# junipertcy/bipartiteSBM-MCMC

Measured on NVIDIA B200. Metric: vertex-moves/sec, higher is better.
Workload: dtype f64+int32

## Files before the change

### bipartitesbm-mcmc_b200/csrc/capi.cu

```cuda
#include "../../include/bisbm.h"

#include <cuda_runtime.h>
#include <dlfcn.h>
#include <nccl.h>

#include <algorithm>
#include <chrono>
#include <cmath>
#include <cstdarg>
#include <cstdio>
#include <cstdlib>
#include <cstring>
#include <map>
#include <set>
#include <memory>
#include <mutex>
#include <numeric>
#include <string>
#include <vector>

#include "ingest.cuh"
#include "replay.cuh"
#include "merge.cuh"
#include "gltable.h"
// ... 48 lines not shown

struct bisbm_handle {
    int device = 0;
    std::shared_ptr<GraphDev> gdev;
    cudaStream_t stream = nullptr;
    cudaEvent_t ev0 = nullptr, ev1 = nullptr;
    int sm_count = 148;
    uint32_t n = 0, na = 0, nb = 0, W = 0, max_degree = 0;
    uint64_t n_edges = 0;
    std::vector<uint32_t> h_row_ptr, h_degvals;
    uint32_t *d_row_ptr = nullptr, *d_col = nullptr, *d_degidx = nullptr;
    double ent_base = 0.0;
    double* d_qtab = nullptr;
    GlNode* d_gl = nullptr;
    uint32_t gl_n = 0;
    uint32_t qn = 0, qk = 0;
    double* d_lg = nullptr;
    uint64_t lg_n = 0;
    uint32_t n_chains = 0, C = 0, KA = 0, KB = 0;
    std::vector<uint32_t> h_ka, h_kb;
    uint32_t *d_ka = nullptr, *d_kb = nullptr;
    int32_t *d_labels = nullptr, *d_labels_tmp = nullptr, *d_m = nullptr, *d_e = nullptr, *d_nr = nullptr,
            *d_eta = nullptr;
    int32_t *d_m2 = nullptr, *d_e2 = nullptr, *d_nr2 = nullptr;
    int32_t* d_nr_live = nullptr;
    int32_t* d_eta_snap = nullptr;
    double* d_kat_out = nullptr;
    ncclComm_t comm = nullptr;
    uint8_t* d_lab8 = nullptr;
    double eps = 1.0;
    LogqExp* d_lq = nullptr;
    uint64_t* d_seeds = nullptr;
    uint8_t* d_active = nullptr;
    unsigned long long *d_accepted = nullptr, *d_u = nullptr, *d_sweeps = nullptr;
    double *d_dS = nullptr, *d_entmin = nullptr, *d_ent_out = nullptr;
    uint32_t* d_nactive = nullptr;
    uint64_t sweep_epoch = 0;
    std::map<uint32_t, ReplaySlot> replay;
    uint32_t* d_hist = nullptr;
    uint32_t hist_width = 0;
    uint32_t al_ka = 0, al_kb = 0, al_segments = 0;
    uint32_t *d_al_order = nullptr, *d_al_seg = nullptr, *d_al_overlap = nullptr, *d_al_map = nullptr;
    bool al_sampled = false;
    double last_ms = 0.0;
    uint64_t last_launches = 0, last_moves = 0;
    int precision = BISBM_PRECISION_FP64;
    int opt_kernel = -1;
    uint32_t opt_inflight_div = 64;
    int opt_generic = 0;
// ... 24 lines not shown
template <typename T>
void dfree(T*& p) {
    if (p) cudaFree(p);
    p = nullptr;
}

void free_ladder(bisbm_handle* h) {
    dfree(h->d_tp_rung_beta); dfree(h->d_tp_beta); dfree(h->d_tp_rung_of); dfree(h->d_tp_chain_at); dfree(h->d_tp_trip);
    dfree(h->d_tp_acc_prev); dfree(h->d_tp_stats);
    h->tp_rungs = 0;
    h->tp_round = 0;
}

void free_align(bisbm_handle* h) {
    dfree(h->d_al_order); dfree(h->d_al_seg); dfree(h->d_al_overlap); dfree(h->d_al_map);
    h->al_ka = h->al_kb = h->al_segments = 0;
    h->al_sampled = false;
}

void free_chains(bisbm_handle* h) {
    free_ladder(h);
    free_align(h);
    dfree(h->d_ka); dfree(h->d_kb); dfree(h->d_labels); dfree(h->d_labels_tmp);
    dfree(h->d_m); dfree(h->d_e); dfree(h->d_nr); dfree(h->d_eta); dfree(h->d_lq); dfree(h->d_m2); dfree(h->d_e2); dfree(h->d_nr2); dfree(h->d_nr_live); dfree(h->d_eta_snap); dfree(h->d_kat_out); dfree(h->d_lab8);
    dfree(h->d_seeds); dfree(h->d_active); dfree(h->d_accepted); dfree(h->d_u); dfree(h->d_sweeps);
    dfree(h->d_dS); dfree(h->d_entmin); dfree(h->d_ent_out); dfree(h->d_nactive); dfree(h->d_hist);
    for (auto& kv : h->replay) { dfree(kv.second.d_rs); dfree(kv.second.d_vlist); dfree(kv.second.d_kh); }
    h->replay.clear();
    h->n_chains = 0;
}

GraphView gview(const bisbm_handle* h) {
    GraphView g;
    g.n = h->n; g.na = h->na; g.nb = h->nb; g.n_edges = h->n_edges;
    g.row_ptr = h->d_row_ptr; g.col = h->d_col; g.degidx = h->d_degidx;
    g.W = h->W; g.max_degree = h->max_degree;
    return g;
}

StateView sview(const bisbm_handle* h) {
    StateView s;
    s.C = h->C; s.KA = h->KA; s.KB = h->KB; s.W = h->W;
    s.labels = h->d_labels; s.m = h->d_m; s.e = h->d_e; s.nr = h->d_nr; s.eta = h->d_eta;
    s.ka = h->d_ka; s.kb = h->d_kb; s.eps = h->eps;
    return s;
}

// ... 436 lines not shown
        if (e != cudaSuccess)
            return fail(BISBM_ERR_CUDA, "sweep_kernel launch failed: %s (kernel %d, grid %u, %d threads, %zu bytes of shared memory)",
                        cudaGetErrorString(e), lp.kernel, grid, NT, lp.smem_bytes);
    }
    return BISBM_OK;
}

template <typename HistT>
int launch_sweep_nt(bisbm_handle* h, const SweepParams& P, const LaunchPlan& lp) {
    if (lp.wpc == 32) return launch_sweep_t<HistT, 1024>(h, P, lp);
    return launch_sweep_t<HistT, 512>(h, P, lp);
}

int launch_sweep_h(bisbm_handle* h, const SweepParams& P, const LaunchPlan& lp) {
    if (lp.hist_bytes == 1) return launch_sweep_nt<uint8_t>(h, P, lp);
    if (lp.hist_bytes == 2) return launch_sweep_nt<uint16_t>(h, P, lp);
    return launch_sweep_nt<uint32_t>(h, P, lp);
}

template <typename R, int KF, int TYPE, bool STAGED = true, int NT = 512>
int launch_sweep2_t(bisbm_handle* h, const SweepParams& P, const LaunchPlan& lp, unsigned grid) {
    int rc = ensure_smem_attr(h, (const void*)sweep2_kernel<R, KF, TYPE, STAGED, NT>, (int)kSmemMax);
    if (rc) return rc;
    sweep2_kernel<R, KF, TYPE, STAGED, NT><<<grid, lp.wpc * 32, lp.smem_bytes, h->stream>>>(P);
    {
        const cudaError_t e = cudaGetLastError();
        if (e != cudaSuccess)
            return fail(BISBM_ERR_CUDA, "sweep2_kernel launch failed: %s (kernel %d, grid %u, %u warps, %zu bytes of shared memory)",
                        cudaGetErrorString(e), lp.kernel, grid, lp.wpc, lp.smem_bytes);
    }
    wrote_labels8(h);
    return BISBM_OK;
}

template <typename R>
int launch_sweep2(bisbm_handle* h, const SweepParams& P, const LaunchPlan& lp, unsigned grid) {
    if (!kern_is_s2(lp.kernel) || lp.wpc > 24) return fail(BISBM_ERR_STATE, "internal: sweep2 launcher with the plan of kernel %d (%u warps)", lp.kernel, lp.wpc);
    if (!lp.smem) return launch_sweep2_t<R, 0, 0, false>(h, P, lp, grid);
    if (h->KA == 32 && h->KB == 32 && !h->opt_generic) {
#ifdef BISBM_WARP_VARIANTS
        if (lp.wpc == 24) return P.type ? launch_sweep2_t<R, 32, 1, true, 768>(h, P, lp, grid) : launch_sweep2_t<R, 32, 0, true, 768>(h, P, lp, grid);
        if (lp.wpc == 20) return P.type ? launch_sweep2_t<R, 32, 1, true, 640>(h, P, lp, grid) : launch_sweep2_t<R, 32, 0, true, 640>(h, P, lp, grid);
#endif
        return P.type ? launch_sweep2_t<R, 32, 1>(h, P, lp, grid) : launch_sweep2_t<R, 32, 0>(h, P, lp, grid);
    }
    return launch_sweep2_t<R, 0, 0>(h, P, lp, grid);
}

__attribute__((noinline)) int dispatch_sweep(bisbm_handle* h, const SweepParams& P, const LaunchPlan& lp, unsigned grid) {
    switch (lp.kernel) {
        case KERN_S2_F64: case KERN_S2L_F64: return launch_sweep2<double>(h, P, lp, grid);
        case KERN_S2_F32: case KERN_S2L_F32: return launch_sweep2<float>(h, P, lp, grid);
        case KERN_L2: {
            const int rc = launch_sweep_h(h, P, lp);
            wrote_labels32(h);
            return rc;
        }
        default: return fail(BISBM_ERR_STATE, "internal: no launcher for kernel %d", lp.kernel);
    }
}

SweepParams base_params(bisbm_handle* h, uint32_t type) {
    SweepParams P;
    memset(&P, 0, sizeof P);
    P.g = gview(h); P.s = sview(h); P.tb = tview(h, false);
    P.lab8 = h->d_lab8; P.m_next = h->d_m2; P.e_next = h->d_e2; P.nr_next = h->d_nr2; P.nr_live = h->d_nr_live;
    P.eta_read = h->d_eta;
    P.seeds = h->d_seeds; P.active = h->d_active; P.accepted = h->d_accepted; P.dS_accum = h->d_dS;
    P.lq = h->d_lq;
    P.n_chains = h->n_chains; P.type = type; P.n_groups = h->C / 32;
    P.kopp_max = type ? h->KA : h->KB;
    P.half_bits = feistel_half_bits(type ? h->nb : h->na);
    P.kat_out = h->d_kat_out;
    P.vary_k = (uint32_t)h->opt_vary_k;
    return P;
}

int launch_full_sweep(bisbm_handle* h, int schedule, float p0, float p1, uint64_t sweep_in_call, uint32_t max_inflight,
                      const double* beta_chain = nullptr) {
    uint32_t wpc = 32;
    const int kernel = plan_kernel(h, &wpc);
    if (!kern_is_s2(kernel)) {
        int rc = sync_labels32(h);
        if (rc) return rc;
    }
    {
        int rc = sync_labels8(h);
        if (rc) return rc;
    }
    for (uint32_t type = 0; type < 2; ++type) {
        const uint32_t nv = type ? h->nb : h->na;
        if (nv == 0) continue;
        LaunchPlan lp;
        int rc = plan_sweep(h, type, max_inflight, kernel, wpc, &lp);
        if (rc) return rc;
        const uint32_t kmax = type ? h->KB : h->KA;
        const uint32_t tot = h->n_chains * kmax;
        logq_refresh_kernel<<<(tot * 16 + 127) / 128, 128, 0, h->stream>>>(sview(h), tview(h, false), h->d_lq, h->n_chains, type);
        h->last_launches += 1;
        const uint32_t n_m = h->C * h->KA * h->KB, n_e = h->C * (h->KA + h->KB);
        const bool sliced = lp.smem && lp.ctas_per_group > 1;
        h->last_wpc = lp.wpc; h->last_cpg = lp.ctas_per_group; h->last_slice = lp.slice;
        h->last_kernel = kernel;
        uint32_t extras = 0;
        const uint32_t G = h->C / 32;
        if (sliced && h->opt_spare_sms && max_inflight == 0 && (uint32_t)h->sm_count > G * lp.ctas_per_group)
            extras = std::min<uint32_t>((uint32_t)h->sm_count - G * lp.ctas_per_group, G - 1);
        const uint32_t per_cta = lp.slice / std::max<uint32_t>(1, lp.ctas_per_group);
        for (uint32_t l = 0;; ++l) {
            const uint64_t pos = extras ? ((uint64_t)l * lp.ctas_per_group + ((uint64_t)l * extras) / G) * per_cta : (uint64_t)l * lp.slice;
            if (pos >= nv) break;
            if (sliced && l != 0 && l % h->opt_logq_every == 0) {
                logq_refresh_kernel<<<(tot * 16 + 127) / 128, 128, 0, h->stream>>>(sview(h), tview(h, false), h->d_lq, h->n_chains, type, 1u);
                h->last_launches += 1;
            }
            if (sliced) {
                const uint32_t nmax = std::max(std::max(n_m, n_e), G * kmax * h->W * 32u);
                sweep2_preinit_kernel<<<(nmax + 255) / 256, 256, 0, h->stream>>>(h->d_m, h->d_e, h->d_nr, h->d_m2, h->d_e2, h->d_nr2,
                                                                                 h->d_nr_live, n_m, n_e, h->KA, h->KB, type, lp.ctas_per_group - 1,
                                                                                 G, extras, l, h->d_eta, h->d_eta_snap, h->W);
                h->last_launches += 1;
            }
            SweepParams P = base_params(h, type);
            if (sliced) P.eta_read = h->d_eta_snap;
            P.ctas_per_group = lp.ctas_per_group; P.warps_used = lp.warps_used;
            P.pos_begin = (uint32_t)pos; P.pos_end = (uint32_t)std::min<uint64_t>(nv, pos + lp.slice);
            P.exclusive = sliced ? 0 : 1;
            P.sweep = h->sweep_epoch;
            P.step_base = sweep_in_call * (uint64_t)h->n + (type ? h->na : 0);
            P.schedule = schedule; P.p0 = p0; P.p1 = p1; P.beta0 = (p0 == 0.0f) ? -1.0 : 1.0 / (double)p0;
            if (schedule == BISBM_ABRUPT_COOL) {
                const uint64_t lo = P.step_base, hi = P.step_base + nv;
                if ((float)(hi - 1) < p0) { P.schedule = BISBM_CONSTANT; P.p0 = 1.0f; P.beta0 = 1.0; }
                else if (!((float)lo < p0)) { P.schedule = BISBM_CONSTANT; P.p0 = 0.0f; P.beta0 = -1.0; }
            }
            P.beta_chain = beta_chain;
            P.extras = extras; P.launch_idx = l; P.per_cta = per_cta;
            const unsigned grid = P.n_groups * lp.ctas_per_group + extras;
            rc = dispatch_sweep(h, P, lp, grid);
            if (rc) return rc;
            h->last_launches += 1;
            h->last_sweep_launches += 1;
            if (sliced) {
                std::swap(h->d_m, h->d_m2); std::swap(h->d_e, h->d_e2); std::swap(h->d_nr, h->d_nr2);
            }
        }
    }
    h->sweep_epoch++;
    h->last_moves += (uint64_t)h->n * h->n_chains;
    return BISBM_OK;
}

int sync_labels8(bisbm_handle* h) {
    if (!h->lab8_stale) return BISBM_OK;
    const uint64_t total = (uint64_t)h->n * h->C;
    const uint64_t threads = (total + 3) / 4;
    labels8_kernel<<<(unsigned)((threads + 255) / 256), 256, 0, h->stream>>>(h->d_labels, h->d_lab8, total);
    CU(cudaGetLastError());
    h->lab8_stale = false;
    return BISBM_OK;
}

int sync_labels32(bisbm_handle* h) {
    if (!h->lab32_stale) return BISBM_OK;
    const uint64_t total = (uint64_t)h->n * h->C;
    const uint64_t threads = (total + 3) / 4;
    labels32_kernel<<<(unsigned)((threads + 255) / 256), 256, 0, h->stream>>>(h->d_lab8, h->d_labels, total);
    CU(cudaGetLastError());
// ... 221 lines not shown
    free_ladder(h);
    free_align(h);
    uint32_t KA = 0, KB = 0;
    for (uint32_t c = 0; c < n_chains; ++c) {
        if (ka[c] == 0 || kb[c] == 0) return fail(BISBM_ERR_ARG, "chain %u: ka and kb must be >= 1", c);
        KA = std::max(KA, ka[c]); KB = std::max(KB, kb[c]);
    }
    KA = std::max(KA, h->opt_reserve_ka); KB = std::max(KB, h->opt_reserve_kb);
    const uint32_t C = (n_chains + 31) / 32 * 32;
    const uint32_t n = h->n;
    const size_t KK = (size_t)KA + KB;
    bool reuse = h->n_chains == n_chains && h->C == C && h->KA == KA && h->KB == KB && h->d_labels;
    bool same_model = reuse && h->eps == eps;
    for (uint32_t c = 0; same_model && c < n_chains; ++c) same_model = h->h_ka[c] == ka[c] && h->h_kb[c] == kb[c];
    if (!reuse) {
        free_chains(h);
        h->n_chains = n_chains; h->C = C; h->KA = KA; h->KB = KB;
        CU(cudaMalloc(&h->d_ka, C * sizeof(uint32_t)));
        CU(cudaMalloc(&h->d_kb, C * sizeof(uint32_t)));
        CU(cudaMalloc(&h->d_labels, (size_t)n * C * sizeof(int32_t)));
        CU(cudaMalloc(&h->d_labels_tmp, (size_t)n * C * sizeof(int32_t)));
        CU(cudaMalloc(&h->d_m, (size_t)C * KA * KB * sizeof(int32_t)));
        CU(cudaMalloc(&h->d_e, (size_t)C * KK * sizeof(int32_t)));
        CU(cudaMalloc(&h->d_m2, (size_t)C * KA * KB * sizeof(int32_t)));
        CU(cudaMalloc(&h->d_e2, (size_t)C * KK * sizeof(int32_t)));
        CU(cudaMalloc(&h->d_lab8, (size_t)n * C));
        CU(cudaMalloc(&h->d_nr, (size_t)C * KK * sizeof(int32_t)));
        CU(cudaMalloc(&h->d_nr2, (size_t)C * KK * sizeof(int32_t)));
        CU(cudaMalloc(&h->d_nr_live, (size_t)C * KK * sizeof(int32_t)));
        CU(cudaMalloc(&h->d_kat_out, 2 * sizeof(double)));
        CU(cudaMalloc(&h->d_eta, (size_t)C * KK * h->W * sizeof(int32_t)));
        CU(cudaMalloc(&h->d_eta_snap, (size_t)C * KK * h->W * sizeof(int32_t)));
        CU(cudaMalloc(&h->d_lq, (size_t)C * KK * sizeof(LogqExp)));
        CU(cudaMalloc(&h->d_seeds, C * sizeof(uint64_t)));
        CU(cudaMalloc(&h->d_active, C));
        CU(cudaMalloc(&h->d_accepted, C * sizeof(unsigned long long)));
        CU(cudaMalloc(&h->d_u, C * sizeof(unsigned long long)));
        CU(cudaMalloc(&h->d_sweeps, C * sizeof(unsigned long long)));
        CU(cudaMalloc(&h->d_dS, C * sizeof(double)));
        CU(cudaMalloc(&h->d_entmin, C * sizeof(double)));
        CU(cudaMalloc(&h->d_ent_out, C * sizeof(double)));
        CU(cudaMalloc(&h->d_nactive, sizeof(uint32_t)));
    } else {
        for (auto& kv : h->replay) { dfree(kv.second.d_rs); dfree(kv.second.d_vlist); dfree(kv.second.d_kh); }
        h->replay.clear();
    }
    h->eps = eps;
    h->h_ka.assign(C, 1); h->h_kb.assign(C, 1);
    std::copy(ka, ka + n_chains, h->h_ka.begin());
    std::copy(kb, kb + n_chains, h->h_kb.begin());
    CU(cudaMemsetAsync(h->d_lq, 0, (size_t)C * KK * sizeof(LogqExp), h->stream));
    CU(cudaMemsetAsync(h->d_dS, 0, C * sizeof(double), h->stream));
    CU(cudaMemsetAsync(h->d_active, 0, C, h->stream));
    CU(cudaMemsetAsync(h->d_active, 1, n_chains, h->stream));
    CU(cudaMemcpyAsync(h->d_ka, h->h_ka.data(), C * sizeof(uint32_t), cudaMemcpyHostToDevice, h->stream));
// ... 1084 lines not shown
    } else if (k == "warps") {
        if (value != 16 && value != 20 && value != 24) return fail(BISBM_ERR_ARG, "warps: 16, 20 or 24");
        h->opt_warps = (uint32_t)value;
    } else if (k == "generic") {
        h->opt_generic = value != 0;
    } else if (k == "logq_every") {
        if (value < 1 || value > 0x7fffffff) return fail(BISBM_ERR_ARG, "logq_every must be >= 1");
        h->opt_logq_every = (uint32_t)value;
    } else if (k == "spare_sms") {
        h->opt_spare_sms = value != 0;
    } else if (k == "reserve_ka" || k == "reserve_kb") {
        if (value < 0 || value > (1 << 20)) return fail(BISBM_ERR_ARG, "%s out of range", name);
        (k == "reserve_ka" ? h->opt_reserve_ka : h->opt_reserve_kb) = (uint32_t)value;
    } else {
        return fail(BISBM_ERR_ARG, "unknown option '%s'", name);
    }
    return BISBM_OK;
}

#ifdef BISBM_ROUND_CLOCKS
int bisbm_round_clocks(unsigned long long* out) {
    if (!out) return fail(BISBM_ERR_ARG, "null argument");
    CU(cudaDeviceSynchronize());
    CU(cudaMemcpyFromSymbol(out, g_round_clocks, sizeof(unsigned long long) * 8));
    const unsigned long long zero[8] = {0, 0, 0, 0, 0, 0, 0, 0};
    CU(cudaMemcpyToSymbol(g_round_clocks, zero, sizeof zero));
    return BISBM_OK;
}
#endif

int bisbm_parallel_transition(bisbm_handle* h, uint32_t chain, uint32_t v, uint32_t s, double* dS, double* log_accu) {
    int rc = need_chains(h);
    if (rc) return rc;
    if (chain >= h->n_chains) return fail(BISBM_ERR_ARG, "chain %u out of range", chain);
    const uint32_t ka = h->h_ka[chain], kb = h->h_kb[chain];
    if (v >= h->n || s >= ka + kb) return fail(BISBM_ERR_ARG, "vertex or block out of range");
    const bool va = v < h->na;
    if ((s < ka) != va) {
        if (dS) *dS = INFINITY;
        if (log_accu) *log_accu = NAN;
        return BISBM_OK;
    }
    uint32_t wpc = 32;
    const int kernel = plan_kernel(h, &wpc);
    if (!kern_is_s2(kernel))
        return fail(BISBM_ERR_STATE, "bisbm_parallel_transition needs the sweep2 kernel (degrees > 255 or K > 256 per type take the round-1 kernel)");
    const uint32_t type = va ? 0 : 1;
    rc = sync_labels8(h);
// ... 320 lines not shown
```

### bipartitesbm-mcmc_b200/csrc/sweep.cuh

```cuda
#pragma once
#include "state.cuh"

namespace bisbm {

struct LogqExp {
    int32_t e0, n0;
    double fe, fn;
    float fee, fen, fnn, feee;
    uint32_t valid, pad;
};

struct SweepParams {
    GraphView g;
    StateView s;
    Tables tb;
    uint8_t* lab8;
    int32_t* m_next;
    int32_t* e_next;
    const uint64_t* seeds;
    const uint8_t* active;
    unsigned long long* accepted;
    double* dS_accum;
    const LogqExp* lq;
    uint32_t n_chains;
    uint32_t type;
    uint32_t n_groups;
    uint32_t ctas_per_group;
    uint32_t warps_used;
    uint32_t pos_begin, pos_end;
    uint32_t half_bits;
    uint32_t kopp_max;
    uint32_t exclusive;
    uint64_t sweep;
    uint64_t step_base;
    int schedule;
    float p0, p1;
    int32_t* nr_next;
    int32_t* nr_live;
    const int32_t* eta_read;
    uint32_t group_offset;
    uint32_t kat_mode;
    uint32_t kat_chain, kat_v, kat_s;
    double* kat_out;
    double beta0;
    uint32_t extras, launch_idx, per_cta;
    uint32_t vary_k;
    const double* beta_chain;
};

BISBM_NOINLINE_HD static double par_temperature(int schedule, float p0, float p1, uint64_t t) {
    switch (schedule) {
        case 0: return (double)p0 * pow((double)p1, (double)t);
        case 1: return (double)(p0 - p1 * (float)t);
        case 2: {
            uint64_t i = (uint64_t)((float)t + p1);
            double l = (i == 0) ? 0.0 : log((double)i);
            return (double)p0 / l;
        }
        case 3: return (double)p0;
        default: return ((float)t < p0) ? 1.0 : 0.0;
    }
}
// ... 440 lines not shown
```

### bipartitesbm-mcmc_b200/csrc/sweep2.cuh

```cuda
#pragma once
#include <string.h>
#include "sweep.cuh"

namespace bisbm {

#if !defined(BISBM_NO_CVT_MAGIC) && !defined(BISBM_CVT_MAGIC)
#define BISBM_CVT_MAGIC 1
#endif

#define BISBM_LN2F 0.69314718055994530942f
#define BISBM_LOG2EF 1.44269504088896340736f

#if defined(__CUDA_ARCH__)
__device__ __forceinline__ float f_lg2(float x) { float y; asm("lg2.approx.ftz.f32 %0, %1;" : "=f"(y) : "f"(x)); return y; }
__device__ __forceinline__ float f_ex2(float x) { float y; asm("ex2.approx.ftz.f32 %0, %1;" : "=f"(y) : "f"(x)); return y; }
__device__ __forceinline__ float f_rcp(float x) { float y; asm("rcp.approx.ftz.f32 %0, %1;" : "=f"(y) : "f"(x)); return y; }
#else
inline float f_lg2(float x) { return log2f(x); }
inline float f_ex2(float x) { return exp2f(x); }
inline float f_rcp(float x) { return 1.0f / x; }
#endif

template <typename R> struct Ar;

// ... 270 lines not shown
__device__ __forceinline__ void bulk_red_add_s32(void* dst, uint32_t src, uint32_t bytes) {
    asm volatile("cp.reduce.async.bulk.global.shared::cta.bulk_group.add.s32 [%0], [%1], %2;"
                 :: "l"(__cvta_generic_to_global(dst)), "r"(src), "r"(bytes) : "memory");
}
__device__ __forceinline__ void bulk_commit_wait_all() {
    asm volatile("cp.async.bulk.commit_group;" ::: "memory");
    asm volatile("cp.async.bulk.wait_group 0;" ::: "memory");
}

__device__ __forceinline__ int gl_ld(uint64_t base, uint32_t off, uint32_t on) {
    int v;
    asm("{\n\t.reg .u64 a;\n\t.reg .pred p;\n\tsetp.ne.u32 p, %3, 0;\n\tcvt.u64.u32 a, %2;\n\tadd.u64 a, a, %1;\n\tmov.s32 %0, 0;\n\t@p ld.global.cg.s32 %0, [a];\n\t}"
        : "=r"(v) : "l"(base), "r"(off), "r"(on));
    return v;
}
__device__ __forceinline__ void gl_red(uint64_t base, uint32_t off, int v) {
    asm volatile("{\n\t.reg .u64 a;\n\tcvt.u64.u32 a, %1;\n\tadd.u64 a, a, %0;\n\tred.global.add.s32 [a], %2;\n\t}" :: "l"(base), "r"(off), "r"(v) : "memory");
}
__device__ __forceinline__ int gl_atom(uint64_t base, uint32_t off, int v) {
    int o; asm volatile("{\n\t.reg .u64 a;\n\tcvt.u64.u32 a, %2;\n\tadd.u64 a, a, %1;\n\tatom.global.add.s32 %0, [a], %3;\n\t}" : "=r"(o) : "l"(base), "r"(off), "r"(v) : "memory"); return o;
}

#ifdef BISBM_ROUND_CLOCKS
__device__ unsigned long long g_round_clocks[8];
#define RC_DECL() long long rc[5] = {0, 0, 0, 0, 0}, rc_t = 0, rc_v0 = 0, rc_pass_max = 0; unsigned long long rc_n = 0, rc_rounds = 0
#define RC_START() (rc_t = clock64())
#define RC_MARK(ph) do { const long long t_ = clock64(); rc[ph] += t_ - rc_t; rc_t = t_; } while (0)
#define RC_VSTART() (rc_v0 = rc[0], ++rc_rounds)
#define RC_PASS() do { RC_MARK(0); rc_pass_max = max(rc_pass_max, rc[0] - rc_v0); ++rc_n; } while (0)
#define RC_ROUND() (++rc_rounds)
#define RC_PUBLISH(on) do { if (on) {                                                                                  \
        for (int k_ = 0; k_ < 5; ++k_) atomicAdd(&g_round_clocks[k_], (unsigned long long)rc[k_]);                    \
        atomicAdd(&g_round_clocks[5], rc_n); atomicMax(&g_round_clocks[6], (unsigned long long)rc_pass_max);          \
        atomicAdd(&g_round_clocks[7], rc_rounds); } } while (0)
#else
#define RC_DECL() do {} while (0)
#define RC_START() ((void)0)
#define RC_MARK(ph) ((void)0)
#define RC_VSTART() ((void)0)
#define RC_PASS() ((void)0)
#define RC_ROUND() ((void)0)
#define RC_PUBLISH(on) ((void)0)
#endif

__device__ __noinline__ static double slow2_block_degree_delta(int e_r, int e_s, int d) { return block_degree_delta(e_r, e_s, d); }
__device__ __noinline__ static double slow2_logq_delta(const Tables tb, int e, int n, int de, int dn) {
    return log_q_tab(tb, e + de, n + dn) - log_q_tab(tb, e, n);
}

__device__ __noinline__ static double slow2_beta(int schedule, float p0, float p1, uint64_t t) {
    const double T = par_temperature(schedule, p0, p1, t);
    return (T == 0.0) ? -1.0 : 1.0 / T;
}

__global__ void sweep2_preinit_kernel(const int32_t* __restrict__ m, const int32_t* __restrict__ e, const int32_t* __restrict__ nr,
                                      int32_t* __restrict__ m2, int32_t* __restrict__ e2, int32_t* __restrict__ nr2,
                                      int32_t* __restrict__ nr_live, uint32_t n_m, uint32_t n_e, uint32_t KA, uint32_t KB,
                                      uint32_t type, uint32_t mult,
                                      uint32_t n_groups, uint32_t extras, uint32_t launch_idx,
                                      const int32_t* __restrict__ eta, int32_t* __restrict__ eta_snap, uint32_t W) {
    const uint32_t i = blockIdx.x * blockDim.x + threadIdx.x;
    {
        const uint32_t kown = type ? KB : KA, per = kown * W * 32u;
        if (i < n_groups * per) {
            const uint32_t g = i / per;
            const size_t j = ((size_t)g * (KA + KB) + (type ? KA : 0u)) * W * 32u + (i - g * per);
            eta_snap[j] = eta[j];
        }
    }
    auto extra_of = [&](uint32_t grp) -> uint32_t {
        if (extras == 0u) return 0u;
        const uint32_t slot0 = (uint32_t)(((uint64_t)launch_idx * extras) % n_groups);
        return ((grp + n_groups - slot0) % n_groups < extras) ? 1u : 0u;
    };
    if (i < n_m) m2[i] = (int32_t)(0u - (mult + extra_of(i / (KA * KB * 32u))) * (uint32_t)m[i]);
    if (i < n_e) {
        const uint32_t slot = (i >> 5) % (KA + KB);
        const bool own = type ? (slot >= KA) : (slot < KA);
        const uint32_t ev = (uint32_t)e[i], nv = (uint32_t)nr[i];
        const uint32_t mg = mult + extra_of(i / ((KA + KB) * 32u));
        e2[i] = (int32_t)(own ? 0u - mg * ev : ev);
        nr2[i] = (int32_t)(own ? 0u - mg * nv : nv);
        nr_live[i] = (int32_t)nv;
    }
}

template <typename R, int KF, int TYPE, bool STAGED = true, int NT = 512>
__global__ void __launch_bounds__(NT, 1) sweep2_kernel(const __grid_constant__ SweepParams P) {
    typedef Ar<R> AR;
    extern __shared__ __align__(128) unsigned char s2_smem[];
    unsigned char* const smem_raw = s2_smem;
    constexpr uint32_t FULL = 0xffffffffu;
    uint32_t lane, warp;
    asm volatile("mov.u32 %0, %%laneid;" : "=r"(lane));
    asm volatile("mov.u32 %0, %%tid.x;" : "=r"(warp));
    warp >>= 5;
    const uint32_t wpc = blockDim.x >> 5;
    const GraphView& G = P.g;
    const uint32_t type = KF ? (uint32_t)TYPE : P.type;
    const uint32_t C = P.s.C, KB = KF ? (uint32_t)KF : P.s.KB, KA = KF ? (uint32_t)KF : P.s.KA, W = P.s.W, KK = KA + KB;
    const uint32_t kown_max = type ? KB : KA, kopp_max = type ? KA : KB;
    const uint32_t cta = blockIdx.x;
    const bool extra_cta = P.extras != 0u && cta >= P.n_groups * P.ctas_per_group;
    const uint32_t slot0 = (uint32_t)(((uint64_t)P.launch_idx * P.extras) % P.n_groups);
    const uint32_t grp0 = extra_cta ? (slot0 + (cta - P.n_groups * P.ctas_per_group)) % P.n_groups : cta % P.n_groups;
    const uint32_t group = P.group_offset + grp0;
    const uint32_t cta_in_group = extra_cta ? P.ctas_per_group : cta / P.n_groups;
    const uint32_t own_off = type ? KA : 0, opp_off = type ? 0 : KA;

    int32_t* const gM = P.s.m + (size_t)group * KA * KB * GROUP;
    int32_t* const gE = P.s.e + (size_t)group * KK * GROUP;
    int32_t* const gNR = P.s.nr + (size_t)group * KK * GROUP;
    int32_t* const gLIVE = P.nr_live + (size_t)group * KK * GROUP + (size_t)own_off * 32;
    int32_t* const gETA = P.s.eta + (size_t)group * KK * W * GROUP + (size_t)own_off * W * 32;
    const int32_t* const gETAr = P.eta_read + (size_t)group * KK * W * GROUP + (size_t)own_off * W * 32;
    const LogqExp* const gLQ = P.lq + ((size_t)group * KK + own_off) * GROUP;

    const uint32_t c = group * 32 + lane;
    const bool live = (c < P.n_chains) && P.active[c];
    const uint32_t cc = (c < P.s.C) ? c : 0;
    const uint32_t ka = P.s.ka[cc], kb = P.s.kb[cc], K = ka + kb;
    const uint32_t kown = type ? kb : ka;
    const R eps = (R)P.s.eps;
    const R epsK32 = (R)(P.s.eps * (double)K * 4294967296.0);

    const Sweep2Layout L = sweep2_layout(KA, KB, type, wpc, (uint32_t)sizeof(R), STAGED);
    const uint32_t sbase = (uint32_t)__cvta_generic_to_shared(smem_raw);
    int32_t* const sM = reinterpret_cast<int32_t*>(smem_raw + L.oM);
    int32_t* const sEo = reinterpret_cast<int32_t*>(smem_raw + L.oEo);
    int32_t* const sNo = reinterpret_cast<int32_t*>(smem_raw + L.oNo);
    int32_t* const sEp = reinterpret_cast<int32_t*>(smem_raw + L.oEp);
    R* const sInv = reinterpret_cast<R*>(smem_raw + L.oInv);
    uint32_t* const sSmall = reinterpret_cast<uint32_t*>(smem_raw + L.oSmall);
    uint4* const sVtx = reinterpret_cast<uint4*>(smem_raw + L.oVtx);
    uint32_t* const sCtr = reinterpret_cast<uint32_t*>(smem_raw + L.oCtl + 16);
    const uint32_t mbar = sbase + L.oCtl;
    const uint32_t hist_words = (kopp_max + 3u) / 4u;

    if (STAGED) {
        if (threadIdx.x == 0) {
            mbar_init(mbar, 1);
            asm volatile("fence.mbarrier_init.release.cluster;" ::: "memory");
        }
        __syncthreads();
        if (threadIdx.x == 0) {
            const uint32_t bM = KA * KB * 128u, bO = kown_max * 128u, bP = kopp_max * 128u;
            mbar_expect_tx(mbar, bM + 2u * bO + bP);
            for (uint32_t off = 0; off < bM; off += 32768u)
                bulk_g2s(sbase + L.oM + off, reinterpret_cast<const char*>(gM) + off, min(32768u, bM - off), mbar);
            bulk_g2s(sbase + L.oEo, gE + own_off * 32, bO, mbar);
            bulk_g2s(sbase + L.oNo, gNR + own_off * 32, bO, mbar);
            bulk_g2s(sbase + L.oEp, gE + opp_off * 32, bP, mbar);
        }
    } else {
        for (uint32_t i = threadIdx.x; i < kopp_max * 32u; i += blockDim.x) sEp[i] = __ldcg(gE + opp_off * 32 + i);
    }
    {
        uint32_t* const hw = reinterpret_cast<uint32_t*>(smem_raw + L.oHist);
        for (uint32_t i = threadIdx.x; i < wpc * hist_words * 32u; i += blockDim.x) hw[i] = 0u;
    }

    const uint32_t nv = type ? G.nb : G.na, v0 = type ? G.na : 0;
    uint32_t cpg = P.ctas_per_group;
    uint32_t pos_begin = P.pos_begin, pos_end = P.pos_end;
    if (P.extras != 0u) {
        const uint64_t s0 = (uint64_t)P.launch_idx * P.extras;
        const uint32_t before = (uint32_t)((s0 + P.n_groups - 1u - grp0) / P.n_groups);
        const bool has_extra = (grp0 + P.n_groups - slot0) % P.n_groups < P.extras;
        cpg += has_extra ? 1u : 0u;
        const uint64_t pb = ((uint64_t)P.launch_idx * P.ctas_per_group + before) * P.per_cta;
        pos_begin = (uint32_t)min(pb, (uint64_t)nv);
        pos_end = (uint32_t)min(pb + (uint64_t)cpg * P.per_cta, (uint64_t)nv);
    }
    const uint32_t span = pos_end - pos_begin;
    const uint32_t cnt = P.kat_mode ? (cta_in_group == 0u ? 1u : 0u)
                                    : ((cta_in_group < cpg && span > cta_in_group) ? (span - cta_in_group + cpg - 1u) / cpg : 0u);
    const uint64_t pkey = (P.sweep * 2 + type) * 0x9E3779B97F4A7C15ull + (uint64_t)group * 0xD1B54A32D192ED03ull;
    auto prepare = [&](uint32_t j0) -> uint32_t {
        const uint32_t nb = (cnt > j0) ? min((uint32_t)S2_VB, cnt - j0) : 0u;
        for (uint32_t i = threadIdx.x; i < nb; i += blockDim.x) {
            uint4 b;
            if (P.kat_mode) b.x = P.kat_v;
            else b.x = v0 + feistel_perm(pos_begin + cta_in_group + (j0 + i) * cpg, nv, P.half_bits, pkey);
            b.y = __ldcg(G.row_ptr + b.x);
            b.z = __ldcg(G.row_ptr + b.x + 1) - b.y;
            b.w = __ldcg(G.degidx + b.x);
            sVtx[i] = b;
        }
        if (threadIdx.x == 0) *sCtr = 0u;
        return nb;
    };
    uint32_t nb = prepare(0);
    if (STAGED) mbar_wait(mbar, 0);
    __syncthreads();
    for (uint32_t i = threadIdx.x; i < kopp_max * 32u; i += blockDim.x) {
        const uint32_t ci = min(group * 32u + (i & 31u), C - 1u);
        const double Kc = (double)(P.s.ka[ci] + P.s.kb[ci]);
        sInv[i] = (R)(1.0 / ((double)sEp[i] + P.s.eps * Kc));
    }
    if (STAGED) {
        const int thresh = P.exclusive ? 0x7fffffff : (int)min(span, 0x7ffffff0u) + 1;
        const uint32_t words = (kown_max + 31u) / 32u;
        for (uint32_t i = threadIdx.x; i < words * 32u; i += blockDim.x) {
            const uint32_t w = i >> 5, l = i & 31u;
            uint32_t bits = 0;
            for (uint32_t b = 0; b < 32u && w * 32u + b < kown_max; ++b)
                if (sNo[(w * 32u + b) * 32u + l] <= thresh) bits |= 1u << b;
            sSmall[i] = bits;
        }
    }
    __syncthreads();

    int occ_own = 0, occ_opp = 0;
    if (P.vary_k) {
        for (uint32_t b = 0; b < kown_max; ++b) occ_own += (__ldcg(gNR + (own_off + b) * 32 + lane) > 0) ? 1 : 0;
// ... 57 lines not shown
            rows[j].x = 0u; rows[j].y = 0u;
            if (rho < dcnt)
                asm volatile("{\n\t.reg .u64 a;\n\tmad.wide.u32 a, %2, %3, %4;\n\tld.global.cg.v2.u32 {%0, %1}, [a];\n\t}"
                             : "=r"(rows[j].x), "=r"(rows[j].y) : "r"(ids[j]), "r"(C), "l"(LAB8 + (uint64_t)((lane & 3u) * 8u)));
        }
    };
    auto store_tile = [&](uint32_t dcnt) {
#pragma unroll
        for (int j = 0; j < 4; ++j) {
            if (8u * j < dcnt) {
                asm volatile("st.shared.v2.u32 [%0], {%1, %2};" :: "r"(tile_st + 256u * j), "r"(rows[j].x), "r"(rows[j].y) : "memory");
            }
        }
    };
    auto lab_ld = [&](uint32_t vtx) -> uint32_t {
        uint32_t x;
        asm volatile("{\n\t.reg .u64 a;\n\tmad.wide.u32 a, %1, %2, %3;\n\tld.global.cg.u8 %0, [a];\n\t}" : "=r"(x) : "r"(vtx), "r"(C), "l"(LAB8 + (uint64_t)lane));
        return x;
    };
    auto lab_st = [&](uint32_t vtx, uint32_t x) {
        asm volatile("{\n\t.reg .u64 a;\n\tmad.wide.u32 a, %0, %1, %2;\n\tst.global.u8 [a], %3;\n\t}" :: "r"(vtx), "r"(C), "l"(LAB8 + (uint64_t)lane), "r"(x) : "memory");
    };
    RC_DECL();
    uint32_t ticket = warp;
    auto pop = [&]() -> uint32_t {
        if constexpr (STAGED) { const uint32_t i = ticket; ticket += P.warps_used; return i; }
        uint32_t i = 0;
        if (lane == 0) i = atomicAdd(sCtr, 1u);
        return __shfl_sync(FULL, i, 0);
    };
    const uint32_t round_threads = P.warps_used * 32u;
    auto round_barrier = [&]() {
        if constexpr (STAGED) asm volatile("bar.sync 1, %0;" :: "r"(round_threads) : "memory");
    };

    for (uint32_t j0 = 0;;) {
        if (warp < P.warps_used) {
            ticket = warp;
            uint32_t rounds = 0;
            RC_START();
            uint32_t nxt = pop();
            uint4 ninfo = make_uint4(0, 0, 0, 0);
            uint32_t r_nxt = 0;
            if (nxt < nb) {
                ninfo = sVtx[nxt];
                load_ids(ninfo.y, min(ninfo.z, 32u));
// ... 187 lines not shown
                    }
                    const R a2 = lh - dS * (beta * AR::inv_unit());
                    const bool go_hot = (a2 > (R)0) || (AR::u01(rw) < AR::ex(a2));
                    go = eval && (T_zero ? (dS < (R)0) : go_hot);
                    if (P.kat_mode) {
                        if (lane == kat_lane && eval) { P.kat_out[0] = (double)dS; P.kat_out[1] = (double)(lh * AR::unit()); }
                        go = false;
                    }
                    if (live && !cross && s == r && !T_zero && n_r != 1 && !P.kat_mode) ++n_acc;
                    RC_MARK(1);
                    round_barrier();
                    RC_MARK(3);
                    if (go && P.vary_k) {
                        no_red(r, -1);
                        occ_own += ((n_s == 0) ? 1 : 0) - ((n_r == 1) ? 1 : 0);
                    } else if (go) {
                        if constexpr (STAGED) {
                            const uint32_t small_r = (sh_ld_u32v(Small_base + (r >> 5) * 128u) >> (r & 31u)) & 1u;
                            if (small_r) {
                                if (P.exclusive) {
                                    const int old = sh_atom_add_s32(No_base + r * 128u, -1);
                                    if (old <= 1) { sh_red_add(No_base + r * 128u, 1); go = false; }
                                } else {
                                    const int old = atomicSub(&gLIVE[r * 32 + lane], 1);
                                    if (old <= 1) { atomicAdd(&gLIVE[r * 32 + lane], 1); go = false; }
                                    else sh_red_add(No_base + r * 128u, -1);
                                }
                            } else {
                                sh_red_add(No_base + r * 128u, -1);
                            }
                        } else {
                            if (n_r > SAFE_NR) no_red(r, -1);
                            else {
                                const int old = gl_atom(gNol, r * 128u, -1);
                                if (old <= 1) { no_red(r, 1); go = false; }
                            }
                        }
                    }
                }
                __syncwarp();

                const bool any_go = __any_sync(FULL, go);
                if (d <= 32u) {
                    if (any_go && (STAGED || go)) {
                        const int g1 = go ? 1 : 0;
                        const uint32_t dMs = Ms - Mr;
                        auto move1 = [&](uint32_t t) { const uint32_t f = Mr + t * ST; m_red(f, -g1); m_red(f + dMs, g1); };
// ... 34 lines not shown
                        if (!P.exclusive && ((sh_ld_u32v(Small_base + (s >> 5) * 128u) >> (s & 31u)) & 1u)) atomicAdd(&gLIVE[s * 32 + lane], 1);
                    atomicSub(&gETA[(r * W + didx) * 32 + lane], 1);
                    atomicAdd(&gETA[(s * W + didx) * 32 + lane], 1);
                    lab_st(v, s);
                    ++n_acc;
                    ds_sum += (double)dS;
                }
                RC_MARK(2);
                round_barrier();
                RC_MARK(4);
            }
            if constexpr (STAGED)
                for (const uint32_t all = (nb + P.warps_used - 1u) / P.warps_used; rounds < all; ++rounds) {
                    RC_ROUND(); round_barrier(); RC_MARK(3); round_barrier(); RC_MARK(4);
                }
        }
        j0 += (uint32_t)S2_VB;
        if (j0 >= cnt) break;
        __syncthreads();
        nb = prepare(j0);
        __syncthreads();
    }
    RC_PUBLISH(STAGED && warp < P.warps_used && lane == 0);
    if (warp < P.warps_used && live) {
        if (n_acc) atomicAdd(&P.accepted[c], (unsigned long long)n_acc);
        if (ds_sum != 0.0) atomicAdd(&P.dS_accum[c], ds_sum);
    }

    asm volatile("fence.proxy.async.shared::cta;" ::: "memory");
    __syncthreads();
    if (P.kat_mode || !STAGED) return;
    if (P.exclusive) {
        copy_i4(gM, sM, KA * KB * 32);
        copy_i4(gE + own_off * 32, sEo, kown_max * 32);
        copy_i4(gNR + own_off * 32, sNo, kown_max * 32);
    } else if (threadIdx.x == 0) {
        char* const nM = reinterpret_cast<char*>(P.m_next + (size_t)group * KA * KB * GROUP);
        const uint32_t bM = KA * KB * 128u, bO = kown_max * 128u;
        for (uint32_t off = 0; off < bM; off += 32768u) bulk_red_add_s32(nM + off, sbase + L.oM + off, min(32768u, bM - off));
        bulk_red_add_s32(P.e_next + (size_t)group * KK * GROUP + own_off * 32, sbase + L.oEo, bO);
        bulk_red_add_s32(P.nr_next + (size_t)group * KK * GROUP + own_off * 32, sbase + L.oNo, bO);
        bulk_commit_wait_all();
    }
}

#endif

}
```

Before: 10.62 billion.

## Fold sliced preinit into sweep kernel with PDL and triple-buffered state

```diff
diff --git a/bipartitesbm-mcmc_b200/csrc/capi.cu b/bipartitesbm-mcmc_b200/csrc/capi.cu
--- a/bipartitesbm-mcmc_b200/csrc/capi.cu
+++ b/bipartitesbm-mcmc_b200/csrc/capi.cu
@@ -94,9 +94,10 @@
     uint32_t *d_ka = nullptr, *d_kb = nullptr;
     int32_t *d_labels = nullptr, *d_labels_tmp = nullptr, *d_m = nullptr, *d_e = nullptr, *d_nr = nullptr,
             *d_eta = nullptr;
-    int32_t *d_m2 = nullptr, *d_e2 = nullptr, *d_nr2 = nullptr;
-    int32_t* d_nr_live = nullptr;
-    int32_t* d_eta_snap = nullptr;
+    int32_t *d_m2 = nullptr, *d_e2 = nullptr, *d_nr2 = nullptr, *d_m3 = nullptr, *d_e3 = nullptr, *d_nr3 = nullptr;
+    int32_t* d_nr_live[2] = {nullptr, nullptr};
+    uint64_t nr_live_pos = 0;
+    int32_t* d_eta_ring = nullptr;
     double* d_kat_out = nullptr;
     ncclComm_t comm = nullptr;
     uint8_t* d_lab8 = nullptr;
@@ -167,7 +168,8 @@
     free_ladder(h);
     free_align(h);
     dfree(h->d_ka); dfree(h->d_kb); dfree(h->d_labels); dfree(h->d_labels_tmp);
-    dfree(h->d_m); dfree(h->d_e); dfree(h->d_nr); dfree(h->d_eta); dfree(h->d_lq); dfree(h->d_m2); dfree(h->d_e2); dfree(h->d_nr2); dfree(h->d_nr_live); dfree(h->d_eta_snap); dfree(h->d_kat_out); dfree(h->d_lab8);
+    dfree(h->d_m); dfree(h->d_e); dfree(h->d_nr); dfree(h->d_eta); dfree(h->d_lq); dfree(h->d_m2); dfree(h->d_e2); dfree(h->d_nr2); dfree(h->d_m3); dfree(h->d_e3); dfree(h->d_nr3);
+    dfree(h->d_nr_live[0]); dfree(h->d_nr_live[1]); dfree(h->d_eta_ring); dfree(h->d_kat_out); dfree(h->d_lab8);
     dfree(h->d_seeds); dfree(h->d_active); dfree(h->d_accepted); dfree(h->d_u); dfree(h->d_sweeps);
     dfree(h->d_dS); dfree(h->d_entmin); dfree(h->d_ent_out); dfree(h->d_nactive); dfree(h->d_hist);
     for (auto& kv : h->replay) { dfree(kv.second.d_rs); dfree(kv.second.d_vlist); dfree(kv.second.d_kh); }
@@ -650,9 +652,20 @@
 int launch_sweep2_t(bisbm_handle* h, const SweepParams& P, const LaunchPlan& lp, unsigned grid) {
     int rc = ensure_smem_attr(h, (const void*)sweep2_kernel<R, KF, TYPE, STAGED, NT>, (int)kSmemMax);
     if (rc) return rc;
-    sweep2_kernel<R, KF, TYPE, STAGED, NT><<<grid, lp.wpc * 32, lp.smem_bytes, h->stream>>>(P);
+    cudaError_t launched = cudaSuccess;
+    if (STAGED && !P.exclusive) {
+        cudaLaunchAttribute at[1];
+        at[0].id = cudaLaunchAttributeProgrammaticStreamSerialization;
+        at[0].val.programmaticStreamSerializationAllowed = 1;
+        cudaLaunchConfig_t cfg = {};
+        cfg.gridDim = dim3(grid); cfg.blockDim = dim3(lp.wpc * 32); cfg.dynamicSmemBytes = lp.smem_bytes; cfg.stream = h->stream;
+        cfg.attrs = at; cfg.numAttrs = 1;
+        launched = cudaLaunchKernelEx(&cfg, sweep2_kernel<R, KF, TYPE, STAGED, NT>, P);
+    } else {
+        sweep2_kernel<R, KF, TYPE, STAGED, NT><<<grid, lp.wpc * 32, lp.smem_bytes, h->stream>>>(P);
+    }
     {
-        const cudaError_t e = cudaGetLastError();
+        const cudaError_t le = cudaGetLastError(), e = launched != cudaSuccess ? launched : le;
         if (e != cudaSuccess)
             return fail(BISBM_ERR_CUDA, "sweep2_kernel launch failed: %s (kernel %d, grid %u, %u warps, %zu bytes of shared memory)",
                         cudaGetErrorString(e), lp.kernel, grid, lp.wpc, lp.smem_bytes);
@@ -692,8 +705,8 @@
     SweepParams P;
     memset(&P, 0, sizeof P);
     P.g = gview(h); P.s = sview(h); P.tb = tview(h, false);
-    P.lab8 = h->d_lab8; P.m_next = h->d_m2; P.e_next = h->d_e2; P.nr_next = h->d_nr2; P.nr_live = h->d_nr_live;
-    P.eta_read = h->d_eta;
+    P.lab8 = h->d_lab8;
+    P.eta_read = h->d_eta; P.eta_commit = h->d_eta;
     P.seeds = h->d_seeds; P.active = h->d_active; P.accepted = h->d_accepted; P.dS_accum = h->d_dS;
     P.lq = h->d_lq;
     P.n_chains = h->n_chains; P.type = type; P.n_groups = h->C / 32;
@@ -726,7 +739,6 @@
         const uint32_t tot = h->n_chains * kmax;
         logq_refresh_kernel<<<(tot * 16 + 127) / 128, 128, 0, h->stream>>>(sview(h), tview(h, false), h->d_lq, h->n_chains, type);
         h->last_launches += 1;
-        const uint32_t n_m = h->C * h->KA * h->KB, n_e = h->C * (h->KA + h->KB);
         const bool sliced = lp.smem && lp.ctas_per_group > 1;
         h->last_wpc = lp.wpc; h->last_cpg = lp.ctas_per_group; h->last_slice = lp.slice;
         h->last_kernel = kernel;
@@ -735,6 +747,9 @@
         if (sliced && h->opt_spare_sms && max_inflight == 0 && (uint32_t)h->sm_count > G * lp.ctas_per_group)
             extras = std::min<uint32_t>((uint32_t)h->sm_count - G * lp.ctas_per_group, G - 1);
         const uint32_t per_cta = lp.slice / std::max<uint32_t>(1, lp.ctas_per_group);
+        const size_t n_eta = (size_t)h->C * (h->KA + h->KB) * h->W;
+        int32_t* const eta_S[3] = {h->d_eta_ring, h->d_eta_ring + n_eta, h->d_eta_ring + 2 * n_eta};
+        int32_t *last_read = nullptr, *last_commit = nullptr;
         for (uint32_t l = 0;; ++l) {
             const uint64_t pos = extras ? ((uint64_t)l * lp.ctas_per_group + ((uint64_t)l * extras) / G) * per_cta : (uint64_t)l * lp.slice;
             if (pos >= nv) break;
@@ -742,15 +757,17 @@
                 logq_refresh_kernel<<<(tot * 16 + 127) / 128, 128, 0, h->stream>>>(sview(h), tview(h, false), h->d_lq, h->n_chains, type, 1u);
                 h->last_launches += 1;
             }
+            SweepParams P = base_params(h, type);
             if (sliced) {
-                const uint32_t nmax = std::max(std::max(n_m, n_e), G * kmax * h->W * 32u);
-                sweep2_preinit_kernel<<<(nmax + 255) / 256, 256, 0, h->stream>>>(h->d_m, h->d_e, h->d_nr, h->d_m2, h->d_e2, h->d_nr2,
-                                                                                 h->d_nr_live, n_m, n_e, h->KA, h->KB, type, lp.ctas_per_group - 1,
-                                                                                 G, extras, l, h->d_eta, h->d_eta_snap, h->W);
-                h->last_launches += 1;
+                P.eta_read = (l == 0) ? h->d_eta : eta_S[(l - 1) % 3];
+                P.eta_commit = eta_S[l % 3];
+                P.eta_zero = eta_S[(l + 1) % 3];
+                P.m_next = h->d_m2; P.e_next = h->d_e2; P.nr_next = h->d_nr2;
+                P.m_zero = h->d_m3; P.e_zero = h->d_e3; P.nr_zero = h->d_nr3;
+                P.nr_live = h->d_nr_live[h->nr_live_pos & 1]; P.nr_live_zero = h->d_nr_live[(h->nr_live_pos + 1) & 1];
+                last_read = (l == 0) ? nullptr : eta_S[(l - 1) % 3];
+                last_commit = P.eta_commit;
             }
-            SweepParams P = base_params(h, type);
-            if (sliced) P.eta_read = h->d_eta_snap;
             P.ctas_per_group = lp.ctas_per_group; P.warps_used = lp.warps_used;
             P.pos_begin = (uint32_t)pos; P.pos_end = (uint32_t)std::min<uint64_t>(nv, pos + lp.slice);
             P.exclusive = sliced ? 0 : 1;
@@ -770,8 +787,17 @@
             h->last_launches += 1;
             h->last_sweep_launches += 1;
             if (sliced) {
-                std::swap(h->d_m, h->d_m2); std::swap(h->d_e, h->d_e2); std::swap(h->d_nr, h->d_nr2);
+                int32_t* t = h->d_m; h->d_m = h->d_m2; h->d_m2 = h->d_m3; h->d_m3 = t;
+                t = h->d_e; h->d_e = h->d_e2; h->d_e2 = h->d_e3; h->d_e3 = t;
+                t = h->d_nr; h->d_nr = h->d_nr2; h->d_nr2 = h->d_nr3; h->d_nr3 = t;
+                h->nr_live_pos += 1;
             }
+        }
+        if (last_commit) {
+            const uint32_t kown = type ? h->KB : h->KA, tot_eta = G * kown * h->W * 32u;
+            eta_publish_kernel<<<(tot_eta + 255) / 256, 256, 0, h->stream>>>(h->d_eta, last_commit, last_read, G, h->KA + h->KB,
+                                                                            type ? h->KA : 0u, kown, h->W);
+            h->last_launches += 1;
         }
     }
     h->sweep_epoch++;
@@ -1039,15 +1065,17 @@
         CU(cudaMalloc(&h->d_labels_tmp, (size_t)n * C * sizeof(int32_t)));
         CU(cudaMalloc(&h->d_m, (size_t)C * KA * KB * sizeof(int32_t)));
         CU(cudaMalloc(&h->d_e, (size_t)C * KK * sizeof(int32_t)));
-        CU(cudaMalloc(&h->d_m2, (size_t)C * KA * KB * sizeof(int32_t)));
-        CU(cudaMalloc(&h->d_e2, (size_t)C * KK * sizeof(int32_t)));
         CU(cudaMalloc(&h->d_lab8, (size_t)n * C));
         CU(cudaMalloc(&h->d_nr, (size_t)C * KK * sizeof(int32_t)));
-        CU(cudaMalloc(&h->d_nr2, (size_t)C * KK * sizeof(int32_t)));
-        CU(cudaMalloc(&h->d_nr_live, (size_t)C * KK * sizeof(int32_t)));
+        for (int32_t** p : {&h->d_m2, &h->d_m3}) CU(cudaMalloc(p, (size_t)C * KA * KB * sizeof(int32_t)));
+        for (int32_t** p : {&h->d_e2, &h->d_e3, &h->d_nr2, &h->d_nr3, &h->d_nr_live[0], &h->d_nr_live[1]})
+            CU(cudaMalloc(p, (size_t)C * KK * sizeof(int32_t)));
         CU(cudaMalloc(&h->d_kat_out, 2 * sizeof(double)));
         CU(cudaMalloc(&h->d_eta, (size_t)C * KK * h->W * sizeof(int32_t)));
-        CU(cudaMalloc(&h->d_eta_snap, (size_t)C * KK * h->W * sizeof(int32_t)));
+        CU(cudaMalloc(&h->d_eta_ring, 3 * (size_t)C * KK * h->W * sizeof(int32_t)));
+        CU(cudaMemsetAsync(h->d_m2, 0, (size_t)C * KA * KB * sizeof(int32_t), h->stream));
+        for (int32_t* p : {h->d_e2, h->d_nr2, h->d_nr_live[0], h->d_nr_live[1]}) CU(cudaMemsetAsync(p, 0, (size_t)C * KK * sizeof(int32_t), h->stream));
+        CU(cudaMemsetAsync(h->d_eta_ring, 0, 3 * (size_t)C * KK * h->W * sizeof(int32_t), h->stream));
         CU(cudaMalloc(&h->d_lq, (size_t)C * KK * sizeof(LogqExp)));
         CU(cudaMalloc(&h->d_seeds, C * sizeof(uint64_t)));
         CU(cudaMalloc(&h->d_active, C));
@@ -2178,8 +2206,8 @@
 int bisbm_round_clocks(unsigned long long* out) {
     if (!out) return fail(BISBM_ERR_ARG, "null argument");
     CU(cudaDeviceSynchronize());
-    CU(cudaMemcpyFromSymbol(out, g_round_clocks, sizeof(unsigned long long) * 8));
-    const unsigned long long zero[8] = {0, 0, 0, 0, 0, 0, 0, 0};
+    CU(cudaMemcpyFromSymbol(out, g_round_clocks, sizeof(unsigned long long) * 11));
+    const unsigned long long zero[11] = {};
     CU(cudaMemcpyToSymbol(g_round_clocks, zero, sizeof zero));
     return BISBM_OK;
 }
diff --git a/bipartitesbm-mcmc_b200/csrc/sweep.cuh b/bipartitesbm-mcmc_b200/csrc/sweep.cuh
--- a/bipartitesbm-mcmc_b200/csrc/sweep.cuh
+++ b/bipartitesbm-mcmc_b200/csrc/sweep.cuh
@@ -38,6 +38,9 @@
     int32_t* nr_next;
     int32_t* nr_live;
     const int32_t* eta_read;
+    int32_t* eta_commit;
+    int32_t* eta_zero;
+    int32_t *m_zero, *e_zero, *nr_zero, *nr_live_zero;
     uint32_t group_offset;
     uint32_t kat_mode;
     uint32_t kat_chain, kat_v, kat_s;
diff --git a/bipartitesbm-mcmc_b200/csrc/sweep2.cuh b/bipartitesbm-mcmc_b200/csrc/sweep2.cuh
--- a/bipartitesbm-mcmc_b200/csrc/sweep2.cuh
+++ b/bipartitesbm-mcmc_b200/csrc/sweep2.cuh
@@ -316,7 +316,7 @@
 }
 
 #ifdef BISBM_ROUND_CLOCKS
-__device__ unsigned long long g_round_clocks[8];
+__device__ unsigned long long g_round_clocks[11];
 #define RC_DECL() long long rc[5] = {0, 0, 0, 0, 0}, rc_t = 0, rc_v0 = 0, rc_pass_max = 0; unsigned long long rc_n = 0, rc_rounds = 0
 #define RC_START() (rc_t = clock64())
 #define RC_MARK(ph) do { const long long t_ = clock64(); rc[ph] += t_ - rc_t; rc_t = t_; } while (0)
@@ -327,6 +327,11 @@
         for (int k_ = 0; k_ < 5; ++k_) atomicAdd(&g_round_clocks[k_], (unsigned long long)rc[k_]);                    \
         atomicAdd(&g_round_clocks[5], rc_n); atomicMax(&g_round_clocks[6], (unsigned long long)rc_pass_max);          \
         atomicAdd(&g_round_clocks[7], rc_rounds); } } while (0)
+#define RC_CTA_DECL() long long rck_ = clock64()
+#define RC_CTA_MARK(slot) do { const long long t_ = clock64();                                                        \
+        if (threadIdx.x == 0) atomicAdd(&g_round_clocks[slot], (unsigned long long)(t_ - rck_)); rck_ = t_; } while (0)
+#define RC_CTA_RESET() (rck_ = clock64())
+#define RC_CTA_END() do { RC_CTA_MARK(9); if (threadIdx.x == 0) atomicAdd(&g_round_clocks[10], 1ull); } while (0)
 #else
 #define RC_DECL() do {} while (0)
 #define RC_START() ((void)0)
@@ -335,6 +340,10 @@
 #define RC_PASS() ((void)0)
 #define RC_ROUND() ((void)0)
 #define RC_PUBLISH(on) ((void)0)
+#define RC_CTA_DECL() do {} while (0)
+#define RC_CTA_MARK(slot) ((void)0)
+#define RC_CTA_RESET() ((void)0)
+#define RC_CTA_END() ((void)0)
 #endif
 
 __device__ __noinline__ static double slow2_block_degree_delta(int e_r, int e_s, int d) { return block_degree_delta(e_r, e_s, d); }
@@ -347,41 +356,51 @@
     return (T == 0.0) ? -1.0 : 1.0 / T;
 }
 
-__global__ void sweep2_preinit_kernel(const int32_t* __restrict__ m, const int32_t* __restrict__ e, const int32_t* __restrict__ nr,
-                                      int32_t* __restrict__ m2, int32_t* __restrict__ e2, int32_t* __restrict__ nr2,
-                                      int32_t* __restrict__ nr_live, uint32_t n_m, uint32_t n_e, uint32_t KA, uint32_t KB,
-                                      uint32_t type, uint32_t mult,
-                                      uint32_t n_groups, uint32_t extras, uint32_t launch_idx,
-                                      const int32_t* __restrict__ eta, int32_t* __restrict__ eta_snap, uint32_t W) {
+__global__ void eta_publish_kernel(int32_t* __restrict__ eta, int32_t* __restrict__ S, int32_t* __restrict__ prev, uint32_t n_groups,
+                                   uint32_t KK, uint32_t own_off, uint32_t kown, uint32_t W) {
+    const uint32_t per = kown * W * 32u;
     const uint32_t i = blockIdx.x * blockDim.x + threadIdx.x;
-    {
-        const uint32_t kown = type ? KB : KA, per = kown * W * 32u;
-        if (i < n_groups * per) {
-            const uint32_t g = i / per;
-            const size_t j = ((size_t)g * (KA + KB) + (type ? KA : 0u)) * W * 32u + (i - g * per);
-            eta_snap[j] = eta[j];
-        }
-    }
-    auto extra_of = [&](uint32_t grp) -> uint32_t {
-        if (extras == 0u) return 0u;
-        const uint32_t slot0 = (uint32_t)(((uint64_t)launch_idx * extras) % n_groups);
-        return ((grp + n_groups - slot0) % n_groups < extras) ? 1u : 0u;
-    };
-    if (i < n_m) m2[i] = (int32_t)(0u - (mult + extra_of(i / (KA * KB * 32u))) * (uint32_t)m[i]);
-    if (i < n_e) {
-        const uint32_t slot = (i >> 5) % (KA + KB);
-        const bool own = type ? (slot >= KA) : (slot < KA);
-        const uint32_t ev = (uint32_t)e[i], nv = (uint32_t)nr[i];
-        const uint32_t mg = mult + extra_of(i / ((KA + KB) * 32u));
-        e2[i] = (int32_t)(own ? 0u - mg * ev : ev);
-        nr2[i] = (int32_t)(own ? 0u - mg * nv : nv);
-        nr_live[i] = (int32_t)nv;
+    if (i >= n_groups * per) return;
+    const uint32_t g = i / per;
+    const size_t j = ((size_t)g * KK + own_off) * W * 32u + (i - g * per);
+    eta[j] = S[j];
+    S[j] = 0;
+    if (prev) prev[j] = 0;
+}
+
+__device__ __noinline__ static void sliced_buffer_work(const SweepParams& P, uint32_t group, uint32_t cta_in_group, uint32_t cpg,
+                                                       uint32_t type, uint32_t KA, uint32_t KB, uint32_t kown, uint32_t W) {
+    const uint32_t KK = KA + KB;
+    const uint32_t t0 = cta_in_group * blockDim.x + threadIdx.x, stride = cpg * blockDim.x;
+    const uint32_t nM = KA * KB * 32u, nE = KK * 32u;
+    const size_t offM = (size_t)group * KA * KB * GROUP, offE = (size_t)group * KK * GROUP;
+    for (uint32_t i = t0; i < nM + 2u * nE; i += stride) {
+        const bool in_m = i < nM, in_e = !in_m && i < nM + nE;
+        const uint32_t j = in_m ? i : (in_e ? i - nM : i - nM - nE);
+        const size_t o = (in_m ? offM : offE) + j;
+        const int32_t* const src = in_m ? P.s.m : (in_e ? P.s.e : P.s.nr);
+        int32_t* const dst = in_m ? P.m_next : (in_e ? P.e_next : P.nr_next);
+        int32_t* const zero = in_m ? P.m_zero : (in_e ? P.e_zero : P.nr_zero);
+        const uint32_t slot = j >> 5;
+        const bool own = in_m || (type ? slot >= KA : slot < KA);
+        const uint32_t a = (uint32_t)__ldcg(src + o);
+        const int32_t add = (int32_t)(own ? 0u - (cpg - 1u) * a : a);
+        if (add != 0) atomicAdd(dst + o, add);
+        zero[o] = 0;
+    }
+    for (uint32_t i = t0; i < nE; i += stride) P.nr_live_zero[offE + i] = 0;
+    const size_t eta_off = (size_t)group * KK * W * GROUP + (size_t)(type ? KA : 0u) * W * 32;
+    for (uint32_t i = t0; i < kown * W * 32u; i += stride) {
+        const int32_t x = __ldcg(P.eta_read + eta_off + i);
+        if (x != 0) atomicAdd(P.eta_commit + eta_off + i, x);
+        P.eta_zero[eta_off + i] = 0;
     }
 }
 
 template <typename R, int KF, int TYPE, bool STAGED = true, int NT = 512>
 __global__ void __launch_bounds__(NT, 1) sweep2_kernel(const __grid_constant__ SweepParams P) {
     typedef Ar<R> AR;
+    RC_CTA_DECL();
     extern __shared__ __align__(128) unsigned char s2_smem[];
     unsigned char* const smem_raw = s2_smem;
     constexpr uint32_t FULL = 0xffffffffu;
@@ -406,8 +425,9 @@
     int32_t* const gE = P.s.e + (size_t)group * KK * GROUP;
     int32_t* const gNR = P.s.nr + (size_t)group * KK * GROUP;
     int32_t* const gLIVE = P.nr_live + (size_t)group * KK * GROUP + (size_t)own_off * 32;
-    int32_t* const gETA = P.s.eta + (size_t)group * KK * W * GROUP + (size_t)own_off * W * 32;
-    const int32_t* const gETAr = P.eta_read + (size_t)group * KK * W * GROUP + (size_t)own_off * W * 32;
+    const size_t eta_off = (size_t)group * KK * W * GROUP + (size_t)own_off * W * 32;
+    int32_t* const gETA = P.eta_commit + eta_off;
+    const int32_t* const gETAr = P.eta_read + eta_off;
     const LogqExp* const gLQ = P.lq + ((size_t)group * KK + own_off) * GROUP;
 
     const uint32_t c = group * 32 + lane;
@@ -431,23 +451,9 @@
     const uint32_t mbar = sbase + L.oCtl;
     const uint32_t hist_words = (kopp_max + 3u) / 4u;
 
-    if (STAGED) {
-        if (threadIdx.x == 0) {
-            mbar_init(mbar, 1);
-            asm volatile("fence.mbarrier_init.release.cluster;" ::: "memory");
-        }
-        __syncthreads();
-        if (threadIdx.x == 0) {
-            const uint32_t bM = KA * KB * 128u, bO = kown_max * 128u, bP = kopp_max * 128u;
-            mbar_expect_tx(mbar, bM + 2u * bO + bP);
-            for (uint32_t off = 0; off < bM; off += 32768u)
-                bulk_g2s(sbase + L.oM + off, reinterpret_cast<const char*>(gM) + off, min(32768u, bM - off), mbar);
-            bulk_g2s(sbase + L.oEo, gE + own_off * 32, bO, mbar);
-            bulk_g2s(sbase + L.oNo, gNR + own_off * 32, bO, mbar);
-            bulk_g2s(sbase + L.oEp, gE + opp_off * 32, bP, mbar);
-        }
-    } else {
-        for (uint32_t i = threadIdx.x; i < kopp_max * 32u; i += blockDim.x) sEp[i] = __ldcg(gE + opp_off * 32 + i);
+    if (STAGED && threadIdx.x == 0) {
+        mbar_init(mbar, 1);
+        asm volatile("fence.mbarrier_init.release.cluster;" ::: "memory");
     }
     {
         uint32_t* const hw = reinterpret_cast<uint32_t*>(smem_raw + L.oHist);
@@ -485,6 +491,23 @@
         return nb;
     };
     uint32_t nb = prepare(0);
+    asm volatile("griddepcontrol.wait;" ::: "memory");
+    __syncthreads();
+    if (STAGED) {
+        if (threadIdx.x == 0) {
+            const uint32_t bM = KA * KB * 128u, bO = kown_max * 128u, bP = kopp_max * 128u;
+            mbar_expect_tx(mbar, bM + 2u * bO + bP);
+            for (uint32_t off = 0; off < bM; off += 32768u)
+                bulk_g2s(sbase + L.oM + off, reinterpret_cast<const char*>(gM) + off, min(32768u, bM - off), mbar);
+            bulk_g2s(sbase + L.oEo, gE + own_off * 32, bO, mbar);
+            bulk_g2s(sbase + L.oNo, gNR + own_off * 32, bO, mbar);
+            bulk_g2s(sbase + L.oEp, gE + opp_off * 32, bP, mbar);
+        }
+    } else {
+        for (uint32_t i = threadIdx.x; i < kopp_max * 32u; i += blockDim.x) sEp[i] = __ldcg(gE + opp_off * 32 + i);
+    }
+    if (STAGED && !P.exclusive && !P.kat_mode) sliced_buffer_work(P, group, cta_in_group, cpg, type, KA, KB, kown_max, W);
+    asm volatile("griddepcontrol.launch_dependents;" ::: "memory");
     if (STAGED) mbar_wait(mbar, 0);
     __syncthreads();
     for (uint32_t i = threadIdx.x; i < kopp_max * 32u; i += blockDim.x) {
@@ -588,6 +611,7 @@
         asm volatile("{\n\t.reg .u64 a;\n\tmad.wide.u32 a, %0, %1, %2;\n\tst.global.u8 [a], %3;\n\t}" :: "r"(vtx), "r"(C), "l"(LAB8 + (uint64_t)lane), "r"(x) : "memory");
     };
     RC_DECL();
+    RC_CTA_MARK(8);
     uint32_t ticket = warp;
     auto pop = [&]() -> uint32_t {
         if constexpr (STAGED) { const uint32_t i = ticket; ticket += P.warps_used; return i; }
@@ -821,7 +845,8 @@
                                     const int old = sh_atom_add_s32(No_base + r * 128u, -1);
                                     if (old <= 1) { sh_red_add(No_base + r * 128u, 1); go = false; }
                                 } else {
-                                    const int old = atomicSub(&gLIVE[r * 32 + lane], 1);
+                                    const int old = atomicSub(&gLIVE[r * 32 + lane], 1) +
+                                                    ldc(P.s.nr + ((size_t)group * KK + own_off + r) * GROUP + lane);
                                     if (old <= 1) { atomicAdd(&gLIVE[r * 32 + lane], 1); go = false; }
                                     else sh_red_add(No_base + r * 128u, -1);
                                 }
@@ -902,6 +927,7 @@
         __syncthreads();
     }
     RC_PUBLISH(STAGED && warp < P.warps_used && lane == 0);
+    RC_CTA_RESET();
     if (warp < P.warps_used && live) {
         if (n_acc) atomicAdd(&P.accepted[c], (unsigned long long)n_acc);
         if (ds_sum != 0.0) atomicAdd(&P.dS_accum[c], ds_sum);
@@ -922,8 +948,9 @@
         bulk_red_add_s32(P.nr_next + (size_t)group * KK * GROUP + own_off * 32, sbase + L.oNo, bO);
         bulk_commit_wait_all();
     }
-}
-
-#endif
-
-}
+    RC_CTA_END();
+}
+
+#endif
+
+}
```

Result: faster. 11.01 billion, median of 6 (+3.7%).
